# ChainSafe/lumenos

Hardware: AMD Instinct MI355X
Metric: prove_eval_seconds_16384x4096 (lower is better)
Workload: dtype u64; 1 GPU; Encode+Commit+InnerProduct(r,b)+QueryCols 16384x4096 LogN=14 L=12 K=2 rhoInv=2 queries=309; parallelism=1 GPU: the whole job resident in HBM

## Files before the change

### lumenos_amd/csrc/lm_common.h

```cpp
#pragma once
#include <hip/hip_runtime.h>

#include <algorithm>
#include <cstdarg>
#include <cstdint>
#include <cstdio>
#include <map>
#include <memory>
#include <mutex>
#include <set>
#include <string>
#include <utility>
#include <vector>

#include "../../include/lumenos_hip.h"
#include "lm_arith.h"
#include "lm_dev.h"

#define LM_MAX_LIMBS LUMEN_MAX_LIMBS

struct lm_modmap {
    uint32_t period;
    uint8_t idx[LM_MAX_LIMBS];
};
// ... 11 lines not shown
struct lm_galois_key {
    lm_dev<u64> d_key;
    lm_dev<uint32_t> d_index;
    lm_dev<uint32_t> d_inv_index;
};

struct lumen_set {
    uint32_t count = 0;
    uint32_t nl = 0;
    uint32_t logw = 0;
    u64 *d = nullptr;
    size_t words = 0;
    bool owner = true;
    lumen_ctx *home = nullptr;
};

struct lm_shared {
    std::recursive_mutex mu;
    lm_dev<tw_t> tw_fwd;
    lm_dev<tw_t> tw_inv;
    std::vector<uint64_t> roots;
    uint32_t fieldN = 0;
    lm_dev<tw_t> scal;
    std::map<uint64_t, lm_galois_key> gkeys;
    std::map<std::string, std::shared_ptr<void>> ext;
};

struct lm_tuning {
    uint32_t ks_batch = 64;
    uint32_t ks_lanes = 0;
    int32_t ks_fused_digits = -1;
    uint32_t ks_close_fused = 1;
    uint32_t ks_c0_fold = 1;
    uint32_t debug = 0;
    uint32_t modup_tgroup = 3, moddown_tgroup = 1;
    uint32_t ks_placement = 6;
    uint32_t batch_chunks = 0;
    uint32_t rccl_shared_device = 0;
};

struct lumen_ctx {
    lm_tuning tune;
    std::recursive_mutex mu;
    std::shared_ptr<lm_shared> sh;
    int device = 0;
    hipStream_t stream = nullptr;
    hipStream_t stream2 = nullptr;
    hipEvent_t ev_fork = nullptr, ev_join = nullptr;
    hipStream_t stream_aux = nullptr;
    hipEvent_t ev_aux = nullptr;
    hipEvent_t ev_xdep = nullptr;
    uint32_t aux_digests = 0;
    const u64 *aux_lo = nullptr, *aux_hi = nullptr;
    uint8_t *aux_host = nullptr;
    size_t aux_host_cap = 0;
    void *stage_host = nullptr;
    size_t stage_cap = 0;
    hipEvent_t ev_stage = nullptr;
    void *io_host[2] = {nullptr, nullptr};
    hipEvent_t ev_io[2] = {nullptr, nullptr};
    uint32_t logN = 0, N = 0, L = 0, K = 0;
    uint64_t T = 0;
    uint64_t mod[LM_MAX_LIMBS] = {0};
    uint64_t psi[LM_MAX_LIMBS] = {0};
    lm_mods mods;
    tw_t ninv[LM_MAX_LIMBS];
// ... 169 lines not shown
```

### lumenos_amd/csrc/lm_ctx.hip

```cpp
#include <cstring>
#include <thread>

#include "lm_ntt_plan.h"

thread_local std::string lm_global_err;

int lm_fail(lumen_ctx *ctx, const char *fmt, ...) {
    char buf[1024];
    va_list ap;
    va_start(ap, fmt);
    vsnprintf(buf, sizeof(buf), fmt, ap);
    va_end(ap);
    if (ctx) ctx->err = buf;
    lm_global_err = buf;
    fprintf(stderr, "[lumenos_hip] error: %s\n", buf);
    return 1;
}

void *lm_scratch(lumen_ctx *ctx, const char *name, size_t bytes) {
    auto &e = ctx->scratch[name];
    if (e && e.count() >= bytes) return e.get();
    if (e) lm_sync_all(ctx);
    return e.alloc(ctx, bytes, name) ? nullptr : e.get();
}
// ... 127 lines not shown
static int ctx_private_init(lumen_ctx *ctx) {
    LM_HIP(ctx, hipSetDevice(ctx->device));
    LM_HIP(ctx, hipStreamCreate(&ctx->stream));
    LM_HIP(ctx, hipStreamCreate(&ctx->stream2));
    LM_HIP(ctx, hipEventCreateWithFlags(&ctx->ev_fork, hipEventDisableTiming));
    LM_HIP(ctx, hipEventCreateWithFlags(&ctx->ev_join, hipEventDisableTiming));
    LM_HIP(ctx, hipStreamCreate(&ctx->stream_aux));
    LM_HIP(ctx, hipEventCreateWithFlags(&ctx->ev_aux, hipEventDisableTiming));
    LM_HIP(ctx, hipEventCreateWithFlags(&ctx->ev_stage, hipEventDisableTiming));
    LM_HIP(ctx, hipEventCreateWithFlags(&ctx->ev_xdep, hipEventDisableTiming));
    LM_HIP(ctx, hipEventCreate(&ctx->tm0));
    LM_HIP(ctx, hipEventCreate(&ctx->tm1));
    return 0;
}

static int tuning_set(lm_tuning &t, const char *name, long v) {
    const std::string n(name ? name : "");
    auto in = [&](long lo, long hi) { return v >= lo && v <= hi; };
    if (n == "LUMEN_KS_BATCH") {
        if (!in(1, 4096)) return 2;
        t.ks_batch = (uint32_t)v;
    } else if (n == "LUMEN_KS_LANES") {
        if (!in(0, 2)) return 2;
        t.ks_lanes = (uint32_t)v;
    } else if (n == "LUMEN_KS_FUSED_DIGITS") {
        if (v > LM_MAX_LIMBS) return 2;
        t.ks_fused_digits = v >= 0 ? (int32_t)v : -1;
    } else if (n == "LUMEN_KS_CLOSE_FUSED") {
        if (!in(0, 1)) return 2;
        t.ks_close_fused = (uint32_t)v;
    } else if (n == "LUMEN_KS_C0_FOLD") {
        if (!in(0, 1)) return 2;
        t.ks_c0_fold = (uint32_t)v;
    } else if (n == "LUMEN_DEBUG") {
        t.debug = v != 0;
    } else if (n == "LUMEN_MODUP_TGROUP") {
        if (!in(1, 31)) return 2;
        t.modup_tgroup = (uint32_t)v;
    } else if (n == "LUMEN_MODDOWN_TGROUP") {
        if (!in(1, 31)) return 2;
        t.moddown_tgroup = (uint32_t)v;
    } else if (n == "LUMEN_KS_PLACEMENT") {
        if (!in(0, 32)) return 2;
        t.ks_placement = (uint32_t)v;
    } else if (n == "LUMEN_BATCH_CHUNKS") {
        if (!in(0, 4096)) return 2;
        t.batch_chunks = (uint32_t)v;
    } else {
        return 1;
    }
    return 0;
}
static void tuning_from_env(lm_tuning &t) {
    for (const char *n : {"LUMEN_KS_BATCH", "LUMEN_KS_LANES", "LUMEN_KS_FUSED_DIGITS", "LUMEN_KS_CLOSE_FUSED", "LUMEN_KS_C0_FOLD", "LUMEN_DEBUG",
                          "LUMEN_MODUP_TGROUP", "LUMEN_MODDOWN_TGROUP", "LUMEN_KS_PLACEMENT", "LUMEN_BATCH_CHUNKS"}) {
        const char *e = getenv(n);
        if (e && *e && tuning_set(t, n, atol(e)))
            fprintf(stderr, "[lumenos_hip] %s=%s is out of range: ignored\n", n, e);
    }
}

extern "C" int lumen_ctx_set_tuning(lumen_ctx *ctx, const char *name, long value) {
    LM_CHECK(nullptr, ctx && name, "lumen_ctx_set_tuning: NULL argument");
    LM_ENTER(ctx);
    const int rc = tuning_set(ctx->tune, name, value);
    LM_CHECK(ctx, rc != 1, "unknown tuning switch %s", name);
    LM_CHECK(ctx, rc == 0, "tuning switch %s: value %ld is out of range (nothing changed)", name, value);
    return 0;
}

extern "C" int lumen_test_allow_shared_device_rccl(lumen_ctx *ctx, int on) {
    LM_CHECK(nullptr, ctx, "lumen_test_allow_shared_device_rccl: NULL ctx");
    LM_ENTER(ctx);
    ctx->tune.rccl_shared_device = on != 0;
    return 0;
}

extern "C" int lumen_ctx_wait(lumen_ctx *ctx, lumen_ctx *other) {
    LM_CHECK(nullptr, ctx && other, "lumen_ctx_wait: NULL argument");
    if (ctx == other) return 0;
    hipEvent_t ev;
    {
        LM_ENTER(other);
        LM_HIP(other, hipEventRecord(other->ev_xdep, other->stream));
        ev = other->ev_xdep;
    }
    LM_ENTER(ctx);
// ... 522 lines not shown
```

### lumenos_amd/csrc/lm_innersum.hip

```cpp
#include <algorithm>

#include "lm_ks_host.h"

__global__ __launch_bounds__(256) void k_acc_canon(u64 *__restrict__ acc, size_t pairs, uint32_t logN, uint32_t L, lm_mods mods) {
    const size_t stride = (size_t)gridDim.x * blockDim.x;
    for (size_t g = (size_t)blockIdx.x * blockDim.x + threadIdx.x; g < pairs; g += stride) {
        const u64 q = mods.m[(uint32_t)((g >> (logN - 1)) % L)].q;
        ulonglong2 v = *reinterpret_cast<ulonglong2 *>(acc + 2 * g);
        v.x = lm_csub(v.x, q), v.y = lm_csub(v.y, q);
        *reinterpret_cast<ulonglong2 *>(acc + 2 * g) = v;
    }
}

__global__ __launch_bounds__(256) void k_lazy_gather(const u64 *__restrict__ u, const u64 *__restrict__ cur, u64 *__restrict__ lazy,
                                                     const uint32_t *__restrict__ index, uint32_t B, uint32_t L, uint32_t K,
                                                     uint32_t pshift, uint32_t logN, uint32_t first, lm_mods mods) {
    const uint32_t N = 1u << logN, nq = L * 2 * B;
    const size_t total = (size_t)2 * B * (L + K) * (N / 2), stride = (size_t)gridDim.x * blockDim.x;
    for (size_t g = (size_t)blockIdx.x * blockDim.x + threadIdx.x; g < total; g += stride) {
        const uint32_t j = (uint32_t)(g & (N / 2 - 1)) * 2, limb = (uint32_t)(g >> (logN - 1));
        const uint32_t t = limb < nq ? limb / (2 * B) : L + (limb - nq) % K;
        const uint32_t pw = limb < nq ? limb % (2 * B) : (limb - nq) / K;
        const bool with_c = t < L && (pw & 1) == (u ? 0u : 1u);
        if (!u && !with_c) continue;
// ... 88 lines not shown
    hipLaunchKernelGGL(k_lazy_gather, dim3(2048), dim3(256), 0, ctx->stream, u, cur, lazy, index, B, tb->nl, ctx->K, ctx->L - tb->nl,
                       ctx->logN, first ? 1u : 0u, ctx->mods);
    LM_HIP(ctx, hipGetLastError());
    return 0;
}

int identity_tables(lumen_ctx *ctx, std::shared_ptr<lm_galois_key> *out) {
    static const char *const NAME = "ks_identity";
    LM_SHARED_LOCK(ctx);
    auto gk = lm_ext_get<lm_galois_key>(ctx, NAME);
    if (!gk) {
        gk = std::make_shared<lm_galois_key>();
        std::vector<uint32_t> index(ctx->N);
        for (uint32_t i = 0; i < ctx->N; i++) index[i] = i;
        if (gk->d_index.upload(ctx, index, "the identity's index table") || gk->d_inv_index.upload(ctx, index, "the identity's index table"))
            return 1;
        lm_ext_put(ctx, NAME, gk);
    }
    *out = std::move(gk);
    return 0;
}

int lazy_close(lumen_ctx *ctx, const u64 *cur, u64 *out, u64 *lazy, uint32_t B, KsTables *tb, const KsScratch &s) {
    std::shared_ptr<lm_galois_key> id;
    if (int rc = identity_tables(ctx, &id)) return rc;
    if (int rc = lazy_gather(ctx, nullptr, cur, lazy, nullptr, false, B, tb)) return rc;
    if (int rc = rotate_p_to_coef(ctx, lazy, B, tb)) return rc;
    KsScratch sl = s;
    sl.u = lazy;
    return rotate_store(ctx, cur, out, B, *id, tb, sl);
}

int inner_sum_batch(lumen_ctx *ctx, u64 *acc, uint32_t B, const SumPlan &plan, KsTables *tb, const KsScratch &s, u64 *lazy,
                    u64 *close_out, u64 *fold_s = nullptr) {
    LM_CHECK(ctx, !close_out || (plan.cnt && !plan.lazy), "InnerSum has no rotation to close");
    LM_CHECK(ctx, !fold_s || (close_out && ks_fold_serves(ctx, tb, plan.cnt)),
             "the c0 fold cannot hold the lifts of %u rotations of %u bits in 192", plan.cnt, tb->lift_bits);
    u64 *cur = acc, *other = s.acc2;
    bool first = true;
    for (uint32_t r = 0; r < plan.cnt; r++) {
        const SumPlan::Step &st = plan.it[r];
        if (int rc = rotate_decompose(ctx, cur, B, tb, s)) return rc;
        if (fold_s) {
            const u64 *s_in = r ? fold_s + ((r - 1) & 1) * ks_fold_words(ctx, B) : nullptr;
            u64 *s_out = fold_s + (r & 1) * ks_fold_words(ctx, B);
            if (r + 1 == plan.cnt) return rotate_close_fold(ctx, cur, close_out, B, *st.dbl, st.dbl_el, tb, s, s_in, s_out);
            if (int rc = rotate_add_fold(ctx, cur, other, B, *st.dbl, st.dbl_el, tb, s, s_in, s_out)) return rc;
            std::swap(cur, other);
            continue;
        }
        if (st.term) {
            if (int rc = rotate_mac(ctx, cur, B, *st.term, tb, s)) return rc;
            if (int rc = lazy_gather(ctx, s.u, cur, lazy, st.term->d_index.get(), first, B, tb)) return rc;
            first = false;
        }
        if (close_out && r + 1 == plan.cnt)
            return rotate_close(ctx, cur, close_out, B, *st.dbl, plan.last_el, tb, s);
        if (int rc = rotate_add(ctx, cur, other, B, *st.dbl, tb, s)) return rc;
        std::swap(cur, other);
    }
    if (plan.lazy) {
        if (int rc = lazy_close(ctx, cur, other, lazy, B, tb, s)) return rc;
        std::swap(cur, other);
    }
    if (cur != acc)
        LM_HIP(ctx, hipMemcpyAsync(acc, cur, (size_t)B * 2 * tb->nl * ctx->N * 8, hipMemcpyDeviceToDevice, ctx->stream));
    return 0;
}

int check_inner_sum_level(lumen_ctx *ctx, const lumen_set *in, const char *what) {
    LM_FULL_WIDTH(ctx, in, what);
    LM_CHECK(ctx, in->nl == ctx->L, "%s is implemented at the top level only (set has %u of %u limbs)", what,
             in->nl, ctx->L);
    return 0;
}

int inner_sum_run(lumen_ctx *ctx, const lumen_set *in, uint32_t batch, uint32_t n, const char *general, lumen_set **out) {
    if (general) {
        if (int rc = general_check(ctx, batch, n, general)) return rc;
    } else {
// ... 33 lines not shown
    }
    KsRun run;
    if (int rc = ks_run_open(ctx, matrix->count, matrix->nl, 2, true, &run)) return rc;
    SumPlan plan;
    if (matrix->count)
        if (int rc = sum_plan(ctx, 1, rows, &plan)) return rc;
    u64 *ptT = nullptr;
    if (int rc = upload_ptT(ctx, pt, matrix->nl, &ptT)) return rc;
    const uint32_t N = ctx->N, L = matrix->nl, target = std::min<uint32_t>(2, L);
    lumen_set *o = nullptr;
    if (int rc = lumen_set_create(ctx, matrix->count, target, &o)) return rc;
    lm_set_guard og(ctx, o);
    const size_t ctw = (size_t)2 * L * N, octw = (size_t)2 * target * N;
    if (int rc = ks_run_scratch(ctx, &run)) return rc;
    u64 *lazy[2] = {nullptr, nullptr};
    if (plan.lazy)
        if (int rc = lazy_blocks(ctx, run, lazy)) return rc;
    u64 *work = (u64 *)lm_scratch(ctx, "rescale_work", run.group_bytes);
    u64 *tbuf = (u64 *)lm_scratch(ctx, "rescale_t", (size_t)run.group * 2 * N * 8);
    if (!work || !tbuf) return 1;
    bool close = false;
    if (L > target && rows > 1 && ctx->tune.ks_close_fused && !plan.lazy && !lm_is_split(ctx->logN)) {
        const int rc = lm_rescale_coef_ready(ctx);
        if (rc && rc != 2) return rc;
        close = rc == 0;
    }
    u64 *fold_s[2] = {nullptr, nullptr};
    if (close && ctx->tune.ks_c0_fold && ks_fold_serves(ctx, run.tb, plan.cnt)) {
        const size_t bytes = 2 * ks_fold_words(ctx, run.Bmax) * 8;
        fold_s[0] = (u64 *)lm_scratch(ctx, "ks_fold_s", bytes);
        fold_s[1] = run.lanes > 1 ? (u64 *)lm_scratch(ctx, "ks_fold_s_b", bytes) : fold_s[0];
        if (!fold_s[0] || !fold_s[1]) return 1;
    }
    auto batch_fn = [&](uint32_t g0, uint32_t first, uint32_t B, const KsScratch &s, u64 *a) {
        if (int rc = launch_mul_plain(ctx, matrix->d + (size_t)(g0 + first) * ctw, a, ptT, (size_t)B * ctw, L, B))
            return rc;
        const int lane = &s == &run.s[1];
        return inner_sum_batch(ctx, a, B, plan, run.tb, s, lazy[lane], close ? work + (size_t)first * ctw : nullptr, fold_s[lane]);
    };
    auto end_of_group = [&](uint32_t g0, uint32_t gn) {
        if (close)
            return lm_rescale_polys_from_coef(ctx, work, L, o->d + (size_t)g0 * octw, target, gn * 2);
        if (L > target) return lm_rescale_polys(ctx, run.acc, L, o->d + (size_t)g0 * octw, target, gn * 2, work, tbuf);
        if (!plan.lazy)
            if (int rc = acc_canon(ctx, run.acc, (size_t)gn * ctw, L)) return rc;
        LM_HIP(ctx, hipMemcpyAsync(o->d + (size_t)g0 * octw, run.acc, (size_t)gn * ctw * 8, hipMemcpyDeviceToDevice, ctx->stream));
        return 0;
    };
    if (int rc = ks_run(ctx, run, matrix->count, ctw, batch_fn, end_of_group)) return rc;
    *out = og.release();
    return 0;
}

}

extern "C" int lumen_inner_sum_general(lumen_ctx *ctx, const lumen_set *in, uint32_t batch_size, uint32_t n, lumen_set **out) {
    LM_CHECK(nullptr, ctx && in && out, "lumen_inner_sum_general: NULL argument");
    LM_ENTER(ctx);
    if (int rc = check_level_of_chain(ctx, in, "InnerSum")) return rc;
    return inner_sum_run(ctx, in, batch_size, n, "lumen_inner_sum_general", out);
}

extern "C" int lumen_matrix_inner_sum_general(lumen_ctx *ctx, const lumen_set *matrix, const uint64_t *pt, uint32_t rows,
                                              lumen_set **out) {
    LM_CHECK(nullptr, ctx && matrix && pt && out, "lumen_matrix_inner_sum_general: NULL argument");
    LM_ENTER(ctx);
    if (int rc = check_level_of_chain(ctx, matrix, "matrixInnerSumEval")) return rc;
    return matrix_inner_sum_run(ctx, matrix, pt, rows, "lumen_matrix_inner_sum_general", out);
}

extern "C" uint32_t lumen_inner_sum_general_elements(const lumen_ctx *ctx, uint32_t batch_size, uint32_t n, uint64_t *gal_els) {
// ... 41 lines not shown
```

### lumenos_amd/csrc/lm_keyswitch.hip

```cpp
#include <cstdlib>
#include <cstring>

#include "lm_ks_host.h"

__device__ __forceinline__ u32 bx_v(u128 A, u128 M, u64 y0, u64 y1, u64 m0, u64 m1) {
    const u128 D1 = A >= M ? A - M : M - A, D2 = 2 * M - A;
    if ((u64)(D1 >> 64) >= 8 && (u64)(D2 >> 64) >= 8) return A >= M ? 1u : 0u;
    double vf = 0.0;
    vf += (double)y0 / (double)m0;
    vf += (double)y1 / (double)m1;
    return (u32)(u64)vf;
}

__device__ __forceinline__ void pack_pair(u64 a, u64 b, u64 m0, u64 m1, u128 M, u64 &hi, u64 &lo) {
    u64 l1, h1, l2, h2;
    mul128(a, m1, l1, h1);
    mul128(b, m0, l2, h2);
    const u128 A = (((u128)h1 << 64) | l1) + (((u128)h2 << 64) | l2);
    const u32 v = bx_v(A, M, a, b, m0, m1);
    const u128 W = A + (v == 0 ? 2 * M : (v == 1 ? M : (u128)0));
    hi = (u64)(W >> LM_W_SPLIT), lo = (u64)W & ((1ull << LM_W_SPLIT) - 1);
}

__global__ __launch_bounds__(256) void k_pack_v(u64 *__restrict__ y, size_t poly_stride, uint32_t npoly,
                                                uint32_t ngroups, uint32_t group_limbs, uint32_t first_mod,
                                                uint32_t nlimbs_total, uint32_t logN, lm_mods mods) {
    const uint32_t N = 1u << logN;
    const size_t total = (size_t)npoly * ngroups * (N / 2), stride = (size_t)gridDim.x * blockDim.x;
    for (size_t g = (size_t)blockIdx.x * blockDim.x + threadIdx.x; g < total; g += stride) {
        const uint32_t i = (uint32_t)(g & (N / 2 - 1)) * 2;
        const uint32_t grp = (uint32_t)((g >> (logN - 1)) % ngroups), p = (uint32_t)((g >> (logN - 1)) / ngroups);
        const uint32_t l0 = grp * group_limbs;
        if (l0 + 1 >= nlimbs_total) continue;
        u64 *y0 = y + (size_t)p * poly_stride + (size_t)l0 * N + i;
        const ulonglong2 av = *reinterpret_cast<const ulonglong2 *>(y0);
        const ulonglong2 bv = *reinterpret_cast<const ulonglong2 *>(y0 + N);
        const u64 m0 = mods.m[first_mod + l0].q, m1 = mods.m[first_mod + l0 + 1].q;
        u64 Ml, Mh;
        mul128(m0, m1, Ml, Mh);
        const u128 M = ((u128)Mh << 64) | Ml;
        ulonglong2 hv, lv;
#pragma unroll
        for (int e = 0; e < 2; e++) {
            const u64 a = e ? av.y : av.x, b = e ? bv.y : bv.x;
            u64 hi, lo;
            pack_pair(a, b, m0, m1, M, hi, lo);
            if (e) hv.y = hi, lv.y = lo;
            else hv.x = hi, lv.x = lo;
        }
        *reinterpret_cast<ulonglong2 *>(y0) = hv;
        *reinterpret_cast<ulonglong2 *>(y0 + N) = lv;
    }
}

template <int LOGN>
// ... 597 lines not shown
    } else {
        if (int rc = lm_launch_ntt_strided(ctx, acc + (size_t)L * N, (size_t)2 * L * N, s.coef, (size_t)L * N, B,
                                           lm_map_q(L), true, "ks_intt_c1", &tb->yscale))
            return rc;
    }
    if (K == 2 && nf < beta) {
        lm_prof_scope ps(ctx, "ks_pack_v", (uint64_t)B);
        if (int rc = lm_launch_pack_v(ctx, s.coef + (size_t)2 * nf * N, (size_t)L * N, B, beta - nf, K, 2 * nf, L - 2 * nf)) return rc;
    }
    {
        const uint64_t nb = (uint64_t)B * tb->pairs.size();
        const uint32_t *work = nullptr;
        if (int rc = modup_work_list(ctx, tb, B, &work)) return rc;
        lm_prof_scope ps(ctx, "ks_modup_ntt", nb);
        if (int rc = lm_for_any_logn(ctx, ctx->logN, [&](auto n) {
                return lm_launch(ctx, k_modup_ntt<n>, lm_geom_fwd(n), lm_fwd_grid<n>((uint32_t)nb), s.coef, acc, s.ext, tb->d_bx.get(), B, L, K, beta,
                                 pshift, work, ctx->mods, ctx->sh->tw_fwd.get());
            }))
            return rc;
    }
    return 0;
}

int rotate_product(lumen_ctx *ctx, const u64 *acc, uint32_t B, const lm_galois_key &gk, KsTables *tb, const KsScratch &s) {
    if (int rc = rotate_mac(ctx, acc, B, gk, tb, s)) return rc;
    return rotate_p_to_coef(ctx, s.u, B, tb);
}

int rotate_mac(lumen_ctx *ctx, const u64 *acc, uint32_t B, const lm_galois_key &gk, KsTables *tb, const KsScratch &s) {
    lm_prof_scope ps(ctx, "ks_mac", (uint64_t)B);
    return launch_ks_mac(ctx, s.ext, acc, gk.d_key.get(), s.u, B, tb);
}

int rotate_p_to_coef(lumen_ctx *ctx, u64 *u, uint32_t B, KsTables *tb) {
    const uint32_t N = ctx->N, L = tb->nl, K = ctx->K;
    u64 *up = u + ks_u_at(0, L, B, L, K) * N;
    const size_t pstride = (size_t)K * N;
    if (int rc = lm_launch_ntt_strided(ctx, up, pstride, up, pstride, B * 2, lm_map_p(ctx), true, "ks_intt_p",
                                       &tb->yscale))
        return rc;
    if (K == 2) {
        lm_prof_scope ps(ctx, "ks_pack_v", (uint64_t)B);
        if (int rc = lm_launch_pack_v(ctx, up, pstride, B * 2, 1u, K, ctx->L, K)) return rc;
    }
    return 0;
}

int rotate_accumulate(lumen_ctx *ctx, const u64 *acc, u64 *acc_out, uint32_t B, const lm_galois_key &gk,
                      KsTables *tb, const KsScratch &s) {
    if (int rc = rotate_decompose(ctx, acc, B, tb, s)) return rc;
    return rotate_add(ctx, acc, acc_out, B, gk, tb, s);
}

int rotate_add(lumen_ctx *ctx, const u64 *acc, u64 *acc_out, uint32_t B, const lm_galois_key &gk, KsTables *tb, const KsScratch &s) {
    if (int rc = rotate_product(ctx, acc, B, gk, tb, s)) return rc;
    return launch_moddown<true>(ctx, acc, acc_out, B, gk, tb, s);
}

int rotate_store(lumen_ctx *ctx, const u64 *in, u64 *out, uint32_t B, const lm_galois_key &gk, KsTables *tb, const KsScratch &s) {
    return launch_moddown<false>(ctx, in, out, B, gk, tb, s);
}

int rotate_close(lumen_ctx *ctx, const u64 *acc, u64 *coef_out, uint32_t B, const lm_galois_key &gk, uint64_t gal_el,
                 KsTables *tb, const KsScratch &s) {
    if (int rc = rotate_product(ctx, acc, B, gk, tb, s)) return rc;
    const uint32_t *work_down = nullptr;
    if (int rc = moddown_work_list(ctx, tb, B, &work_down)) return rc;
    return ks_close_launch(ctx, acc, coef_out, B, gk, gal_el, tb, s, work_down);
}

#ifndef LM_KS_FOLD_MIN_ROTATIONS
#define LM_KS_FOLD_MIN_ROTATIONS 3
#endif
bool ks_fold_serves(const lumen_ctx *ctx, const KsTables *tb, uint32_t rotations) {
    return ctx->N >= 256 && !lm_is_split(ctx->logN) && ctx->K >= 1 && ctx->K <= 2 && rotations >= LM_KS_FOLD_MIN_ROTATIONS &&
           rotations + tb->lift_bits <= 191;
}

int rotate_add_fold(lumen_ctx *ctx, const u64 *acc, u64 *acc_out, uint32_t B, const lm_galois_key &gk, uint64_t gal_el, KsTables *tb,
                    const KsScratch &s, const u64 *s_in, u64 *s_out) {
    {
        lm_prof_scope ps(ctx, "ks_mac", (uint64_t)B);
        if (int rc = launch_ks_mac_fold(ctx, s.ext, acc, gk, s.u, acc_out, B, tb)) return rc;
    }
    if (int rc = rotate_p_to_coef(ctx, s.u, B, tb)) return rc;
    if (int rc = lift_fold_launch(ctx, s.u, s_in, s_out, B, gal_el, tb)) return rc;
    return launch_moddown<true>(ctx, acc, acc_out, B, gk, tb, s, true);
}

int rotate_close_fold(lumen_ctx *ctx, const u64 *acc, u64 *coef_out, uint32_t B, const lm_galois_key &gk, uint64_t gal_el,
                      KsTables *tb, const KsScratch &s, const u64 *s_in, u64 *s_out) {
    if (int rc = rotate_product(ctx, acc, B, gk, tb, s)) return rc;
    if (int rc = lift_fold_launch(ctx, s.u, s_in, s_out, B, gal_el, tb)) return rc;
    const uint32_t *work_down = nullptr;
    if (int rc = moddown_work_list(ctx, tb, B, &work_down)) return rc;
    return ks_close_launch(ctx, acc, coef_out, B, gk, gal_el, tb, s, work_down, s_out);
}

extern "C" int lumen_ks_mac_probe(lumen_ctx *ctx, uint32_t batch, const void *ext, const void *acc, const void *key,
                                  void *u, uint32_t reps, float *ms_per_launch) {
    LM_CHECK(nullptr, ctx && ms_per_launch, "lumen_ks_mac_probe: NULL argument");
    LM_ENTER(ctx);
    KsTables *tb = nullptr;
    if (int rc = get_tables(ctx, &tb)) return rc;
    const uint32_t N = ctx->N, L = ctx->L, B = batch ? batch : ks_batch(ctx);
    LM_CHECK(ctx, B <= 65535 && reps >= 1 && reps <= 100000, "lumen_ks_mac_probe: batch %u / reps %u out of range", B, reps);
    KsScratch s;
    if (int rc = get_scratch(ctx, B, tb, &s)) return rc;
    if (!acc) acc = lm_scratch(ctx, "ks_acc", (size_t)B * 2 * L * N * 8);
    if (!acc) return 1;
    if (!key) {
        LM_SHARED_LOCK(ctx);
        LM_CHECK(ctx, !ctx->gkeys.empty(), "lumen_ks_mac_probe: no Galois key loaded");
        key = ctx->gkeys.begin()->second.d_key.get();
    }
    const u64 *pe = ext ? (const u64 *)ext : s.ext;
    u64 *pu = u ? (u64 *)u : s.u;
    auto launch = [&] { return launch_ks_mac(ctx, pe, (const u64 *)acc, (const u64 *)key, pu, B, tb); };
    for (int i = 0; i < 3; i++)
        if (int rc = launch()) return rc;
    LM_HIP(ctx, hipEventRecord(ctx->tm0, ctx->stream));
    for (uint32_t i = 0; i < reps; i++)
        if (int rc = launch()) return rc;
    LM_HIP(ctx, hipEventRecord(ctx->tm1, ctx->stream));
    LM_HIP(ctx, hipEventSynchronize(ctx->tm1));
    float ms = 0;
    LM_HIP(ctx, hipEventElapsedTime(&ms, ctx->tm0, ctx->tm1));
    *ms_per_launch = ms / (float)reps;
// ... 3 lines not shown
```

### lumenos_amd/csrc/lm_ks_close.hip

```cpp
#include "lm_ks_host.h"

#ifndef LM_KS_CLOSE_PF
#define LM_KS_CLOSE_PF 4
#endif

template <int LOGN, bool FOLD>
__global__ LM_GEOM_BOUNDS(lm_geom_lds(LOGN)) void k_ks_close(const u64 *__restrict__ u, const u64 *__restrict__ acc_in,
                                                              u64 *__restrict__ out, const bx_t *__restrict__ bxp,
                                                              const tw_t *__restrict__ pinv,
                                                              const uint32_t *__restrict__ index,
                                                              const uint32_t *__restrict__ inv_index, uint32_t ginv,
                                                              const uint32_t *__restrict__ work, uint32_t B, uint32_t L,
                                                              uint32_t K, lm_mods mods, lm_ninv_t ninv,
                                                              const tw_t *__restrict__ tw_all,
                                                              const u64 *__restrict__ fold_s,
                                                              const sfold_t *__restrict__ sfc) {
    extern __shared__ __attribute__((aligned(16))) u64 sm[];
    constexpr uint32_t N = 1u << LOGN;
    const uint32_t tid = threadIdx.x;
    const uint32_t wk = work[blockIdx.x];
    const uint32_t pw = wk & 0xFFFF;
    const uint32_t t = wk >> 16;
    const uint32_t w = pw & 1;
    const bx_t c = bxp[t];
// ... 74 lines not shown
                const u64 m = lm_shoup3<true>(bx_apply(c, h, l, qc), npi.w, npi.wp, qc.nq);
                y = r + (src(i) >= N ? qc.q3 - m : m);
            }
            y = lm_csub(lm_csub(y, 4 * qc.q), 2 * qc.q);
            o[i] = lm_csub(y, qc.q);
        }
    } st{o, up0, up1, c, qc, ninv.t[t], npi, ginv, FOLD && w == 0 ? fold_s + (size_t)(pw >> 1) * 3 * N : nullptr, FOLD ? sfc[t] : sfold_t{}, {}, {}, {}};
    lm_ntt_inverse<LOGN>(sm, tw_all + (size_t)t * N, qc, tid, ld, st);
}

static uint32_t inv_mod_2n(uint64_t g, uint32_t N) {
    uint64_t x = g;
    for (int i = 0; i < 5; i++) x *= 2 - g * x;
    return (uint32_t)(x & (2ull * N - 1));
}

int ks_close_launch(lumen_ctx *ctx, const u64 *acc, u64 *out, uint32_t B, const lm_galois_key &gk, uint64_t gal_el,
                    KsTables *tb, const KsScratch &s, const uint32_t *work_down, const u64 *fold_s) {
    const uint32_t L = tb->nl, K = ctx->K;
    const uint32_t ginv = inv_mod_2n(gal_el, ctx->N);
    lm_prof_scope ps(ctx, "rescale_intt", (uint64_t)B * 2 * L);
    return lm_for_logn(ctx, ctx->logN, [&](auto n) {
        constexpr int LN = decltype(n)::value;
        auto go = [&](auto kernel) {
            return lm_launch(ctx, kernel, lm_geom_lds(LN), B * 2 * L, s.u, acc, out, tb->d_bxp.get(), tb->d_pinv.get(), gk.d_index.get(),
                             gk.d_inv_index.get(), ginv, work_down, B, L, K, ctx->mods, lm_ninv_of(ctx), ctx->sh->tw_inv.get(), fold_s,
                             tb->d_sfold.get());
        };
        return fold_s ? go(k_ks_close<LN, true>) : go(k_ks_close<LN, false>);
    });
}

__global__ __launch_bounds__(256) void k_lift_fold(const u64 *__restrict__ up, const u64 *__restrict__ s_in, u64 *__restrict__ s_out,
                                                   uint32_t ginv, uint32_t B, uint32_t K, uint32_t logN, u64 m2_lo, u64 m2_hi) {
    const uint32_t N = 1u << logN, C = N >> 8;
    uint32_t b, chunk;
    if (B % 8 == 0) {
        const uint32_t xcd = blockIdx.x & 7, j = blockIdx.x >> 3;
        b = (j / C) * 8 + xcd, chunk = j % C;
    } else {
        b = blockIdx.x / C, chunk = blockIdx.x % C;
    }
    {
        const uint32_t i = chunk * 256 + threadIdx.x;
        const uint32_t e = (ginv * i) & (2 * N - 1), s = e & (N - 1);
        const u64 *w = up + ((size_t)2 * b * K << logN);
        lm_s192 d;
        if (K == 2) {
            const u64 hi = w[s], lo = w[N + s];
            d = lm_s192_add(lm_s192{lo | (hi << LM_W_SPLIT), hi >> (64 - LM_W_SPLIT), 0}, lm_s192_neg(lm_s192{m2_lo, m2_hi, 0}));
        } else {
            d = lm_s192{w[s], 0, 0};
        }
        const u64 *pi = s_in ? s_in + (size_t)b * 3 * N : nullptr;
        u64 *po = s_out + (size_t)b * 3 * N;
        if (s_in) d = lm_s192_add(d, lm_s192{pi[s], pi[N + s], pi[2 * N + s]});
        if (e >= N) d = lm_s192_neg(d);
        if (s_in) d = lm_s192_add(d, lm_s192{pi[i], pi[N + i], pi[2 * N + i]});
        po[i] = d.a, po[N + i] = d.b, po[2 * N + i] = d.c;
    }
}

int lift_fold_launch(lumen_ctx *ctx, const u64 *u, const u64 *s_in, u64 *s_out, uint32_t B, uint64_t gal_el, KsTables *tb) {
    const uint32_t L = tb->nl, K = ctx->K;
    LM_CHECK(ctx, s_out && s_out != s_in, "the folded lifts need a block of their own");
    LM_CHECK(ctx, ctx->N >= 256, "the lift fold works on blocks of 256 coefficients");
    lm_prof_scope ps(ctx, "ks_lift_fold", (uint64_t)B);
    hipLaunchKernelGGL(k_lift_fold, dim3(B * (ctx->N / 256)), dim3(256), 0, ctx->stream,
                       u + ks_u_at(0, L, B, L, K) * ctx->N, s_in, s_out, inv_mod_2n(gal_el, ctx->N), B, K, ctx->logN, tb->m2_lo, tb->m2_hi);
    LM_HIP(ctx, hipGetLastError());
    return 0;
}
```

### lumenos_amd/csrc/lm_ks_dev.h

```cpp
#pragma once
#include "lm_ntt_dev.h"

struct bx_t {
    tw_t b57;
    u64 c_t;
    uint32_t ns;
    uint32_t own;
};
#define LM_W_SPLIT 57

__device__ __forceinline__ u64 bx_apply(const bx_t &c, u64 a, u64 b, const lm_qc &qc) {
    if (c.ns == 1) return lm_shoup3<true>(a, 1ull, qc.qinv64, qc.nq);
    return lm_shoup3<true>(a, c.b57.w, c.b57.wp, qc.nq, b + c.c_t);
}

struct lm_s192 {
    u64 a, b, c;
};
__host__ __device__ __forceinline__ lm_s192 lm_s192_add(const lm_s192 &x, const lm_s192 &y) {
    lm_s192 r;
    r.a = x.a + y.a;
    const u64 c0 = r.a < x.a ? 1u : 0u;
    r.b = x.b + y.b;
    u64 c1 = r.b < x.b ? 1u : 0u;
// ... 9 lines not shown
    tw_t r64, r128;
    u64 off, pad;
};
__device__ __forceinline__ u64 lm_s192_mod(const sfold_t &f, u64 s0, u64 s1, u64 s2, const lm_qc &qc) {
    const u64 r0 = lm_shoup3<true>(s0, 1ull, qc.qinv64, qc.nq);
    const u64 r1 = lm_shoup3<true>(s1, f.r64.w, f.r64.wp, qc.nq);
    const u64 r2 = lm_shoup3<true>(s2 ^ (1ull << 63), f.r128.w, f.r128.wp, qc.nq);
    return r0 + r1 + r2 + f.off;
}

__host__ __device__ __forceinline__ size_t ks_ext_at(uint32_t b, uint32_t d, uint32_t t, uint32_t B, uint32_t beta) {
    return ((size_t)t * B + b) * beta + d;
}
__host__ __device__ __forceinline__ size_t ks_u_at(uint32_t pw, uint32_t t, uint32_t B, uint32_t L, uint32_t K) {
    return t < L ? (size_t)t * 2 * B + pw : (size_t)L * 2 * B + (size_t)pw * K + (t - L);
}
__host__ __device__ __forceinline__ size_t ks_key_at(uint32_t d, uint32_t w, uint32_t t, uint32_t beta) {
    return ((size_t)t * beta + d) * 2 + w;
}

__host__ __device__ __forceinline__ uint32_t ks_mod_at(uint32_t t, uint32_t nl, uint32_t pshift) {
    return t < nl ? t : t + pshift;
}

__device__ __forceinline__ void mul128(u64 a, u64 b, u64 &lo, u64 &hi) {
    const u32 a0 = (u32)a, a1 = (u32)(a >> 32), b0 = (u32)b, b1 = (u32)(b >> 32);
    const u64 p0 = (u64)a0 * b0;
    const u64 p1 = lm_keep((u64)a0 * b1 + (p0 >> 32));
    const u64 p2 = lm_keep((u64)a1 * b0 + (u32)p1);
    hi = (u64)a1 * b1 + (p1 >> 32) + (p2 >> 32);
    lo = (p2 << 32) | (u32)p0;
}

struct lm_ks_view {
    const bx_t *d_bxp;
    const tw_t *d_pinv;
    const lm_ninv_t *yscale;
};
int lm_ks_tables_view(lumen_ctx *ctx, lm_ks_view *out);
int lm_launch_pack_v(lumen_ctx *ctx, u64 *y, size_t poly_stride, uint32_t npoly, uint32_t ngroups,
                     uint32_t group_limbs, uint32_t first_mod, uint32_t nlimbs_total);
```

### lumenos_amd/csrc/lm_ks_host.h

```cpp
#pragma once
#include "lm_ks_dev.h"

struct KsTables {
    lm_dev<bx_t> d_bx;
    lm_dev<bx_t> d_bxp;
    lm_dev<tw_t> d_pinv;
    lm_dev<sfold_t> d_sfold;
    u64 m2_lo = 0, m2_hi = 0;
    uint32_t lift_bits = 0;
    uint32_t nl = 0;
    uint32_t beta = 0;
    lm_ninv_t yscale;
    std::vector<uint16_t> pairs;
    std::map<uint32_t, lm_dev<uint32_t>> d_work;
    std::map<uint32_t, lm_dev<uint32_t>> d_work_down;
};
int get_tables(lumen_ctx *ctx, KsTables **out);
int get_tables_at(lumen_ctx *ctx, uint32_t nl, KsTables **out);

struct KsScratch {
    u64 *coef, *ext, *u, *acc2;
};

int rotate_decompose(lumen_ctx *ctx, const u64 *acc, uint32_t B, KsTables *tb, const KsScratch &s);
int rotate_product(lumen_ctx *ctx, const u64 *acc, uint32_t B, const lm_galois_key &gk, KsTables *tb, const KsScratch &s);
int rotate_mac(lumen_ctx *ctx, const u64 *acc, uint32_t B, const lm_galois_key &gk, KsTables *tb, const KsScratch &s);
int rotate_p_to_coef(lumen_ctx *ctx, u64 *u, uint32_t B, KsTables *tb);
int rotate_add(lumen_ctx *ctx, const u64 *acc, u64 *acc_out, uint32_t B, const lm_galois_key &gk, KsTables *tb, const KsScratch &s);
int rotate_accumulate(lumen_ctx *ctx, const u64 *acc, u64 *acc_out, uint32_t B, const lm_galois_key &gk,
                      KsTables *tb, const KsScratch &s);
int rotate_store(lumen_ctx *ctx, const u64 *in, u64 *out, uint32_t B, const lm_galois_key &gk, KsTables *tb, const KsScratch &s);
int rotate_close(lumen_ctx *ctx, const u64 *acc, u64 *coef_out, uint32_t B, const lm_galois_key &gk, uint64_t gal_el,
                 KsTables *tb, const KsScratch &s);
int ks_close_launch(lumen_ctx *ctx, const u64 *acc, u64 *out, uint32_t B, const lm_galois_key &gk, uint64_t gal_el,
                    KsTables *tb, const KsScratch &s, const uint32_t *work_down, const u64 *fold_s = nullptr);

bool ks_fold_serves(const lumen_ctx *ctx, const KsTables *tb, uint32_t rotations);
inline size_t ks_fold_words(const lumen_ctx *ctx, uint32_t B) { return (size_t)B * 3 * ctx->N; }
int rotate_add_fold(lumen_ctx *ctx, const u64 *acc, u64 *acc_out, uint32_t B, const lm_galois_key &gk, uint64_t gal_el, KsTables *tb,
                    const KsScratch &s, const u64 *s_in, u64 *s_out);
int rotate_close_fold(lumen_ctx *ctx, const u64 *acc, u64 *coef_out, uint32_t B, const lm_galois_key &gk, uint64_t gal_el,
                      KsTables *tb, const KsScratch &s, const u64 *s_in, u64 *s_out);
int lift_fold_launch(lumen_ctx *ctx, const u64 *u, const u64 *s_in, u64 *s_out, uint32_t B, uint64_t gal_el, KsTables *tb);
int get_scratch(lumen_ctx *ctx, uint32_t B, KsTables *tb, KsScratch *s, int lane = 0, u64 **group_acc = nullptr,
                size_t group_acc_bytes = 0);

int upload_ptT(lumen_ctx *ctx, const uint64_t *pt, uint32_t nl, u64 **out);
int launch_mul_plain(lumen_ctx *ctx, const u64 *ct, u64 *out, const u64 *ptT, size_t words, uint32_t nl,
                     uint32_t ncts);

std::shared_ptr<lm_galois_key> lm_relin_key(lumen_ctx *ctx);
int ks_find_key(lumen_ctx *ctx, uint64_t gal_el, const lm_galois_key **gk);
int check_level_of_chain(lumen_ctx *ctx, const lumen_set *in, const char *what);
uint32_t ks_batch(const lumen_ctx *ctx);
uint32_t ks_lanes(const lumen_ctx *ctx);
struct LaneGuard {
    lumen_ctx *ctx;
    hipStream_t saved;
    LaneGuard(lumen_ctx *c, int lane) : ctx(c), saved(c->stream) {
        if (lane) ctx->stream = ctx->stream2;
    }
    ~LaneGuard() { ctx->stream = saved; }
};

struct KsRun {
    KsTables *top = nullptr, *tb = nullptr;
    uint32_t Bmax = 0, group = 0, lanes = 1;
    bool grouped = false;
    size_t group_bytes = 0;
    KsScratch s[2] = {};
    u64 *acc = nullptr;
};
int ks_run_open(lumen_ctx *ctx, uint32_t count, uint32_t nl, uint32_t max_lanes, bool group_acc, KsRun *run);
int ks_run_scratch(lumen_ctx *ctx, KsRun *run);
template <class Batch, class Group>
int ks_run(lumen_ctx *ctx, const KsRun &run, uint32_t count, size_t ctw, Batch &&batch, Group &&end_of_group) {
// ... 25 lines not shown
```

Measured before the change: 1.629 s.

## Pack only c1 in fold path and overlap lift fold on side stream

In the folded keyswitch path, the pack_v step now runs only over the c1 half, and k_lift_fold does its own pair packing of c0 in-kernel via pack_pair, which is moved into a shared header. An optional FoldSide helper can also put the lift-fold kernel on the second stream with fork/join events so it overlaps the moddown kernels. The side-stream overlap sits behind a new tuning switch that is off by default. The packing change is always active and trades a separate pass over c0 for extra 128-bit arithmetic inside the lift fold.

After: 1.621 s (median of 6 runs). Within noise of the previous version (-0.5%).

```diff
diff --git a/lumenos_amd/csrc/lm_common.h b/lumenos_amd/csrc/lm_common.h
--- a/lumenos_amd/csrc/lm_common.h
+++ b/lumenos_amd/csrc/lm_common.h
@@ -67,6 +67,7 @@
     int32_t ks_fused_digits = -1;
     uint32_t ks_close_fused = 1;
     uint32_t ks_c0_fold = 1;
+    uint32_t ks_fold_side = 0;
     uint32_t debug = 0;
     uint32_t modup_tgroup = 3, moddown_tgroup = 1;
     uint32_t ks_placement = 6;
diff --git a/lumenos_amd/csrc/lm_ctx.hip b/lumenos_amd/csrc/lm_ctx.hip
--- a/lumenos_amd/csrc/lm_ctx.hip
+++ b/lumenos_amd/csrc/lm_ctx.hip
@@ -183,6 +183,9 @@
     } else if (n == "LUMEN_KS_C0_FOLD") {
         if (!in(0, 1)) return 2;
         t.ks_c0_fold = (uint32_t)v;
+    } else if (n == "LUMEN_KS_FOLD_SIDE") {
+        if (!in(0, 1)) return 2;
+        t.ks_fold_side = (uint32_t)v;
     } else if (n == "LUMEN_DEBUG") {
         t.debug = v != 0;
     } else if (n == "LUMEN_MODUP_TGROUP") {
@@ -203,7 +206,8 @@
     return 0;
 }
 static void tuning_from_env(lm_tuning &t) {
-    for (const char *n : {"LUMEN_KS_BATCH", "LUMEN_KS_LANES", "LUMEN_KS_FUSED_DIGITS", "LUMEN_KS_CLOSE_FUSED", "LUMEN_KS_C0_FOLD", "LUMEN_DEBUG",
+    for (const char *n : {"LUMEN_KS_BATCH", "LUMEN_KS_LANES", "LUMEN_KS_FUSED_DIGITS", "LUMEN_KS_CLOSE_FUSED", "LUMEN_KS_C0_FOLD", "LUMEN_KS_FOLD_SIDE",
+                          "LUMEN_DEBUG",
                           "LUMEN_MODUP_TGROUP", "LUMEN_MODDOWN_TGROUP", "LUMEN_KS_PLACEMENT", "LUMEN_BATCH_CHUNKS"}) {
         const char *e = getenv(n);
         if (e && *e && tuning_set(t, n, atol(e)))
diff --git a/lumenos_amd/csrc/lm_innersum.hip b/lumenos_amd/csrc/lm_innersum.hip
--- a/lumenos_amd/csrc/lm_innersum.hip
+++ b/lumenos_amd/csrc/lm_innersum.hip
@@ -144,20 +144,22 @@
 }
 
 int inner_sum_batch(lumen_ctx *ctx, u64 *acc, uint32_t B, const SumPlan &plan, KsTables *tb, const KsScratch &s, u64 *lazy,
-                    u64 *close_out, u64 *fold_s = nullptr) {
+                    u64 *close_out, u64 *fold_s = nullptr, bool fold_side = false) {
     LM_CHECK(ctx, !close_out || (plan.cnt && !plan.lazy), "InnerSum has no rotation to close");
     LM_CHECK(ctx, !fold_s || (close_out && ks_fold_serves(ctx, tb, plan.cnt)),
              "the c0 fold cannot hold the lifts of %u rotations of %u bits in 192", plan.cnt, tb->lift_bits);
     u64 *cur = acc, *other = s.acc2;
     bool first = true;
+    FoldSide side_state(ctx);
+    FoldSide *side = fold_s && fold_side ? &side_state : nullptr;
     for (uint32_t r = 0; r < plan.cnt; r++) {
         const SumPlan::Step &st = plan.it[r];
         if (int rc = rotate_decompose(ctx, cur, B, tb, s)) return rc;
         if (fold_s) {
             const u64 *s_in = r ? fold_s + ((r - 1) & 1) * ks_fold_words(ctx, B) : nullptr;
             u64 *s_out = fold_s + (r & 1) * ks_fold_words(ctx, B);
-            if (r + 1 == plan.cnt) return rotate_close_fold(ctx, cur, close_out, B, *st.dbl, st.dbl_el, tb, s, s_in, s_out);
-            if (int rc = rotate_add_fold(ctx, cur, other, B, *st.dbl, st.dbl_el, tb, s, s_in, s_out)) return rc;
+            if (r + 1 == plan.cnt) return rotate_close_fold(ctx, cur, close_out, B, *st.dbl, st.dbl_el, tb, s, s_in, s_out, side);
+            if (int rc = rotate_add_fold(ctx, cur, other, B, *st.dbl, st.dbl_el, tb, s, s_in, s_out, side)) return rc;
             std::swap(cur, other);
             continue;
         }
@@ -257,11 +259,13 @@
         fold_s[1] = run.lanes > 1 ? (u64 *)lm_scratch(ctx, "ks_fold_s_b", bytes) : fold_s[0];
         if (!fold_s[0] || !fold_s[1]) return 1;
     }
+    const bool fold_side = ctx->tune.ks_fold_side && run.lanes == 1 && ctx->stream != ctx->stream2;
     auto batch_fn = [&](uint32_t g0, uint32_t first, uint32_t B, const KsScratch &s, u64 *a) {
         if (int rc = launch_mul_plain(ctx, matrix->d + (size_t)(g0 + first) * ctw, a, ptT, (size_t)B * ctw, L, B))
             return rc;
         const int lane = &s == &run.s[1];
-        return inner_sum_batch(ctx, a, B, plan, run.tb, s, lazy[lane], close ? work + (size_t)first * ctw : nullptr, fold_s[lane]);
+        return inner_sum_batch(ctx, a, B, plan, run.tb, s, lazy[lane], close ? work + (size_t)first * ctw : nullptr, fold_s[lane],
+                               fold_side);
     };
     auto end_of_group = [&](uint32_t g0, uint32_t gn) {
         if (close)
diff --git a/lumenos_amd/csrc/lm_keyswitch.hip b/lumenos_amd/csrc/lm_keyswitch.hip
--- a/lumenos_amd/csrc/lm_keyswitch.hip
+++ b/lumenos_amd/csrc/lm_keyswitch.hip
@@ -2,25 +2,6 @@
 #include <cstring>
 
 #include "lm_ks_host.h"
-
-__device__ __forceinline__ u32 bx_v(u128 A, u128 M, u64 y0, u64 y1, u64 m0, u64 m1) {
-    const u128 D1 = A >= M ? A - M : M - A, D2 = 2 * M - A;
-    if ((u64)(D1 >> 64) >= 8 && (u64)(D2 >> 64) >= 8) return A >= M ? 1u : 0u;
-    double vf = 0.0;
-    vf += (double)y0 / (double)m0;
-    vf += (double)y1 / (double)m1;
-    return (u32)(u64)vf;
-}
-
-__device__ __forceinline__ void pack_pair(u64 a, u64 b, u64 m0, u64 m1, u128 M, u64 &hi, u64 &lo) {
-    u64 l1, h1, l2, h2;
-    mul128(a, m1, l1, h1);
-    mul128(b, m0, l2, h2);
-    const u128 A = (((u128)h1 << 64) | l1) + (((u128)h2 << 64) | l2);
-    const u32 v = bx_v(A, M, a, b, m0, m1);
-    const u128 W = A + (v == 0 ? 2 * M : (v == 1 ? M : (u128)0));
-    hi = (u64)(W >> LM_W_SPLIT), lo = (u64)W & ((1ull << LM_W_SPLIT) - 1);
-}
 
 __global__ __launch_bounds__(256) void k_pack_v(u64 *__restrict__ y, size_t poly_stride, uint32_t npoly,
                                                 uint32_t ngroups, uint32_t group_limbs, uint32_t first_mod,
@@ -684,7 +665,7 @@
     return launch_ks_mac(ctx, s.ext, acc, gk.d_key.get(), s.u, B, tb);
 }
 
-int rotate_p_to_coef(lumen_ctx *ctx, u64 *u, uint32_t B, KsTables *tb) {
+int rotate_p_to_coef(lumen_ctx *ctx, u64 *u, uint32_t B, KsTables *tb, bool c1_only) {
     const uint32_t N = ctx->N, L = tb->nl, K = ctx->K;
     u64 *up = u + ks_u_at(0, L, B, L, K) * N;
     const size_t pstride = (size_t)K * N;
@@ -693,7 +674,9 @@
         return rc;
     if (K == 2) {
         lm_prof_scope ps(ctx, "ks_pack_v", (uint64_t)B);
-        if (int rc = lm_launch_pack_v(ctx, up, pstride, B * 2, 1u, K, ctx->L, K)) return rc;
+        if (int rc = c1_only ? lm_launch_pack_v(ctx, up + pstride, 2 * pstride, B, 1u, K, ctx->L, K)
+                             : lm_launch_pack_v(ctx, up, pstride, B * 2, 1u, K, ctx->L, K))
+            return rc;
     }
     return 0;
 }
@@ -730,22 +713,29 @@
 }
 
 int rotate_add_fold(lumen_ctx *ctx, const u64 *acc, u64 *acc_out, uint32_t B, const lm_galois_key &gk, uint64_t gal_el, KsTables *tb,
-                    const KsScratch &s, const u64 *s_in, u64 *s_out) {
+                    const KsScratch &s, const u64 *s_in, u64 *s_out, FoldSide *side) {
+    if (side)
+        if (int rc = side->join()) return rc;
     {
         lm_prof_scope ps(ctx, "ks_mac", (uint64_t)B);
         if (int rc = launch_ks_mac_fold(ctx, s.ext, acc, gk, s.u, acc_out, B, tb)) return rc;
     }
-    if (int rc = rotate_p_to_coef(ctx, s.u, B, tb)) return rc;
-    if (int rc = lift_fold_launch(ctx, s.u, s_in, s_out, B, gal_el, tb)) return rc;
+    if (int rc = rotate_p_to_coef(ctx, s.u, B, tb, true)) return rc;
+    if (int rc = lift_fold_launch(ctx, s.u, s_in, s_out, B, gal_el, tb, side)) return rc;
     return launch_moddown<true>(ctx, acc, acc_out, B, gk, tb, s, true);
 }
 
 int rotate_close_fold(lumen_ctx *ctx, const u64 *acc, u64 *coef_out, uint32_t B, const lm_galois_key &gk, uint64_t gal_el,
-                      KsTables *tb, const KsScratch &s, const u64 *s_in, u64 *s_out) {
-    if (int rc = rotate_product(ctx, acc, B, gk, tb, s)) return rc;
-    if (int rc = lift_fold_launch(ctx, s.u, s_in, s_out, B, gal_el, tb)) return rc;
+                      KsTables *tb, const KsScratch &s, const u64 *s_in, u64 *s_out, FoldSide *side) {
+    if (side)
+        if (int rc = side->join()) return rc;
+    if (int rc = rotate_mac(ctx, acc, B, gk, tb, s)) return rc;
+    if (int rc = rotate_p_to_coef(ctx, s.u, B, tb, true)) return rc;
+    if (int rc = lift_fold_launch(ctx, s.u, s_in, s_out, B, gal_el, tb, side)) return rc;
     const uint32_t *work_down = nullptr;
     if (int rc = moddown_work_list(ctx, tb, B, &work_down)) return rc;
+    if (side)
+        if (int rc = side->join()) return rc;
     return ks_close_launch(ctx, acc, coef_out, B, gk, gal_el, tb, s, work_down, s_out);
 }
 
diff --git a/lumenos_amd/csrc/lm_ks_close.hip b/lumenos_amd/csrc/lm_ks_close.hip
--- a/lumenos_amd/csrc/lm_ks_close.hip
+++ b/lumenos_amd/csrc/lm_ks_close.hip
@@ -130,7 +130,8 @@
 }
 
 __global__ __launch_bounds__(256) void k_lift_fold(const u64 *__restrict__ up, const u64 *__restrict__ s_in, u64 *__restrict__ s_out,
-                                                   uint32_t ginv, uint32_t B, uint32_t K, uint32_t logN, u64 m2_lo, u64 m2_hi) {
+                                                   uint32_t ginv, uint32_t B, uint32_t K, uint32_t logN, u64 m0, u64 m1, u64 m2_lo,
+                                                   u64 m2_hi) {
     const uint32_t N = 1u << logN, C = N >> 8;
     uint32_t b, chunk;
     if (B % 8 == 0) {
@@ -145,7 +146,9 @@
         const u64 *w = up + ((size_t)2 * b * K << logN);
         lm_s192 d;
         if (K == 2) {
-            const u64 hi = w[s], lo = w[N + s];
+            const u128 M = (((u128)m2_hi << 64) | m2_lo) >> 1;
+            u64 hi, lo;
+            pack_pair(w[s], w[N + s], m0, m1, M, hi, lo);
             d = lm_s192_add(lm_s192{lo | (hi << LM_W_SPLIT), hi >> (64 - LM_W_SPLIT), 0}, lm_s192_neg(lm_s192{m2_lo, m2_hi, 0}));
         } else {
             d = lm_s192{w[s], 0, 0};
@@ -159,13 +162,36 @@
     }
 }
 
-int lift_fold_launch(lumen_ctx *ctx, const u64 *u, const u64 *s_in, u64 *s_out, uint32_t B, uint64_t gal_el, KsTables *tb) {
+int FoldSide::fork() {
+    LM_HIP(ctx, hipEventRecord(ctx->ev_fork, ctx->stream));
+    LM_HIP(ctx, hipStreamWaitEvent(ctx->stream2, ctx->ev_fork, 0));
+    pending = true;
+    return 0;
+}
+int FoldSide::join() {
+    if (!pending) return 0;
+    pending = false;
+    LM_HIP(ctx, hipEventRecord(ctx->ev_join, ctx->stream2));
+    LM_HIP(ctx, hipStreamWaitEvent(ctx->stream, ctx->ev_join, 0));
+    return 0;
+}
+
+int lift_fold_launch(lumen_ctx *ctx, const u64 *u, const u64 *s_in, u64 *s_out, uint32_t B, uint64_t gal_el, KsTables *tb,
+                     FoldSide *side) {
     const uint32_t L = tb->nl, K = ctx->K;
     LM_CHECK(ctx, s_out && s_out != s_in, "the folded lifts need a block of their own");
     LM_CHECK(ctx, ctx->N >= 256, "the lift fold works on blocks of 256 coefficients");
-    lm_prof_scope ps(ctx, "ks_lift_fold", (uint64_t)B);
-    hipLaunchKernelGGL(k_lift_fold, dim3(B * (ctx->N / 256)), dim3(256), 0, ctx->stream,
-                       u + ks_u_at(0, L, B, L, K) * ctx->N, s_in, s_out, inv_mod_2n(gal_el, ctx->N), B, K, ctx->logN, tb->m2_lo, tb->m2_hi);
+    if (side)
+        if (int rc = side->fork()) return rc;
+    hipStream_t main_stream = ctx->stream;
+    if (side) ctx->stream = ctx->stream2;
+    {
+        lm_prof_scope ps(ctx, "ks_lift_fold", (uint64_t)B);
+        hipLaunchKernelGGL(k_lift_fold, dim3(B * (ctx->N / 256)), dim3(256), 0, ctx->stream, u + ks_u_at(0, L, B, L, K) * ctx->N, s_in,
+                           s_out, inv_mod_2n(gal_el, ctx->N), B, K, ctx->logN, ctx->mod[ctx->L], K == 2 ? ctx->mod[ctx->L + 1] : 0,
+                           tb->m2_lo, tb->m2_hi);
+    }
+    ctx->stream = main_stream;
     LM_HIP(ctx, hipGetLastError());
     return 0;
 }
diff --git a/lumenos_amd/csrc/lm_ks_dev.h b/lumenos_amd/csrc/lm_ks_dev.h
--- a/lumenos_amd/csrc/lm_ks_dev.h
+++ b/lumenos_amd/csrc/lm_ks_dev.h
@@ -65,6 +65,25 @@
     lo = (p2 << 32) | (u32)p0;
 }
 
+__device__ __forceinline__ u32 bx_v(u128 A, u128 M, u64 y0, u64 y1, u64 m0, u64 m1) {
+    const u128 D1 = A >= M ? A - M : M - A, D2 = 2 * M - A;
+    if ((u64)(D1 >> 64) >= 8 && (u64)(D2 >> 64) >= 8) return A >= M ? 1u : 0u;
+    double vf = 0.0;
+    vf += (double)y0 / (double)m0;
+    vf += (double)y1 / (double)m1;
+    return (u32)(u64)vf;
+}
+
+__device__ __forceinline__ void pack_pair(u64 a, u64 b, u64 m0, u64 m1, u128 M, u64 &hi, u64 &lo) {
+    u64 l1, h1, l2, h2;
+    mul128(a, m1, l1, h1);
+    mul128(b, m0, l2, h2);
+    const u128 A = (((u128)h1 << 64) | l1) + (((u128)h2 << 64) | l2);
+    const u32 v = bx_v(A, M, a, b, m0, m1);
+    const u128 W = A + (v == 0 ? 2 * M : (v == 1 ? M : (u128)0));
+    hi = (u64)(W >> LM_W_SPLIT), lo = (u64)W & ((1ull << LM_W_SPLIT) - 1);
+}
+
 struct lm_ks_view {
     const bx_t *d_bxp;
     const tw_t *d_pinv;
diff --git a/lumenos_amd/csrc/lm_ks_host.h b/lumenos_amd/csrc/lm_ks_host.h
--- a/lumenos_amd/csrc/lm_ks_host.h
+++ b/lumenos_amd/csrc/lm_ks_host.h
@@ -25,7 +25,7 @@
 int rotate_decompose(lumen_ctx *ctx, const u64 *acc, uint32_t B, KsTables *tb, const KsScratch &s);
 int rotate_product(lumen_ctx *ctx, const u64 *acc, uint32_t B, const lm_galois_key &gk, KsTables *tb, const KsScratch &s);
 int rotate_mac(lumen_ctx *ctx, const u64 *acc, uint32_t B, const lm_galois_key &gk, KsTables *tb, const KsScratch &s);
-int rotate_p_to_coef(lumen_ctx *ctx, u64 *u, uint32_t B, KsTables *tb);
+int rotate_p_to_coef(lumen_ctx *ctx, u64 *u, uint32_t B, KsTables *tb, bool c1_only = false);
 int rotate_add(lumen_ctx *ctx, const u64 *acc, u64 *acc_out, uint32_t B, const lm_galois_key &gk, KsTables *tb, const KsScratch &s);
 int rotate_accumulate(lumen_ctx *ctx, const u64 *acc, u64 *acc_out, uint32_t B, const lm_galois_key &gk,
                       KsTables *tb, const KsScratch &s);
@@ -37,11 +37,22 @@
 
 bool ks_fold_serves(const lumen_ctx *ctx, const KsTables *tb, uint32_t rotations);
 inline size_t ks_fold_words(const lumen_ctx *ctx, uint32_t B) { return (size_t)B * 3 * ctx->N; }
+struct FoldSide {
+    lumen_ctx *ctx;
+    bool pending = false;
+    explicit FoldSide(lumen_ctx *c) : ctx(c) {}
+    FoldSide(const FoldSide &) = delete;
+    FoldSide &operator=(const FoldSide &) = delete;
+    ~FoldSide() { (void)join(); }
+    int fork();
+    int join();
+};
 int rotate_add_fold(lumen_ctx *ctx, const u64 *acc, u64 *acc_out, uint32_t B, const lm_galois_key &gk, uint64_t gal_el, KsTables *tb,
-                    const KsScratch &s, const u64 *s_in, u64 *s_out);
+                    const KsScratch &s, const u64 *s_in, u64 *s_out, FoldSide *side = nullptr);
 int rotate_close_fold(lumen_ctx *ctx, const u64 *acc, u64 *coef_out, uint32_t B, const lm_galois_key &gk, uint64_t gal_el,
-                      KsTables *tb, const KsScratch &s, const u64 *s_in, u64 *s_out);
-int lift_fold_launch(lumen_ctx *ctx, const u64 *u, const u64 *s_in, u64 *s_out, uint32_t B, uint64_t gal_el, KsTables *tb);
+                      KsTables *tb, const KsScratch &s, const u64 *s_in, u64 *s_out, FoldSide *side = nullptr);
+int lift_fold_launch(lumen_ctx *ctx, const u64 *u, const u64 *s_in, u64 *s_out, uint32_t B, uint64_t gal_el, KsTables *tb,
+                     FoldSide *side = nullptr);
 int get_scratch(lumen_ctx *ctx, uint32_t B, KsTables *tb, KsScratch *s, int lane = 0, u64 **group_acc = nullptr,
                 size_t group_acc_bytes = 0);
 
```
